# raphaelsty/mkb

Hardware: AMD Instinct MI355X
Metric: scored triples/sec (pos+K neg), FB15k-237 RotatE d=1000 (higher is better)
Workload: dtype f32

## Files before the change

### mkb_amd/csrc/score_pool_tile.h

```cpp
#pragma once
#include "score_pool_kernels.h"

namespace mkb {

#ifndef MKB_TILE_KC
#define MKB_TILE_KC 16
#endif
#ifndef MKB_TILE_CP_PIPE
#define MKB_TILE_CP_PIPE 1
#endif
constexpr int kTileKC = MKB_TILE_KC;
constexpr int kTileNQ = kTileKC / 16;
constexpr int kTileRows = 64, kTilePos = 64;
constexpr int kTilePitch = kTileRows * 4 + 4;

struct TileArgs {
    float *part;
    int Kd, ks;
    int fringe_tiles, fringe_slices;
    int row_tiles, pos_tiles;
};

constexpr int kTileL2 = 16;
template <> struct ModelTraits<kTileL2> { static constexpr bool cplx_query = false, cplx_pair = false, uses_gamma = false; };

template <int MODEL, bool HEAD>
__device__ __forceinline__ f2 tile_pair_term(float4 q, float4 x) {
    if constexpr (ModelTraits<MODEL>::cplx_pair) {
        return pair_term_cmod2(f2{q.x, q.y}, f2{q.z, q.w}, f2{x.x, x.y}, f2{x.z, x.w});
    } else {
        static_assert(MODEL == MKB_TRANSE, "real-valued tile: TransE's |q - x| only");
        const f2 a = HEAD ? f2{x.x, x.y} + f2{q.x, q.y} : f2{q.x, q.y} - f2{x.x, x.y};
        const f2 b = HEAD ? f2{x.z, x.w} + f2{q.z, q.w} : f2{q.z, q.w} - f2{x.z, x.w};
        f2 r;
        asm("v_add_f32 %0, |%1|, |%2|" : "=v"(r.x) : "v"(a.x), "v"(b.x));
        asm("v_add_f32 %0, |%1|, |%2|" : "=v"(r.y) : "v"(a.y), "v"(b.y));
        return r;
    }
}

template <int MODEL, bool HEAD>
__device__ __forceinline__ void tile_pair_acc(f2 &acc, float4 q, float4 x) {
    if constexpr (MODEL == kTileL2) {
        const f2 a = f2{q.x, q.y} - f2{x.x, x.y};
        const f2 b = f2{q.z, q.w} - f2{x.z, x.w};
        acc = __builtin_elementwise_fma(b, b, __builtin_elementwise_fma(a, a, acc));
    } else {
        acc += tile_pair_term<MODEL, HEAD>(q, x);
    }
}

template <int MODEL, bool HEAD, int KPT>
__global__ __launch_bounds__(256) void pool_fwd_tile_kernel(PoolArgs A, TileArgs T) {
    constexpr bool CP = ModelTraits<MODEL>::cplx_pair;
    extern __shared__ __attribute__((aligned(16))) int lds_tile_dyn[];
    const int b = (int)blockIdx.x;
    const int n_fringe = T.fringe_tiles * T.fringe_slices;
    if constexpr (MODEL != kTileL2) {
        if (b < n_fringe) {
            pool_fwd_body<MODEL, HEAD, KPT, 4>(A, b % T.fringe_tiles, T.fringe_tiles, b / T.fringe_tiles, T.fringe_slices, lds_tile_dyn);
            return;
        }
    }
    __shared__ __attribute__((aligned(16))) float sq[2][kTileKC / 2][kTilePitch];
    __shared__ __attribute__((aligned(16))) float sx[2][kTileKC / 2][kTilePitch];
    int t = b - n_fringe;
    const int z = t % T.ks; t /= T.ks;
    const int i0 = (t % T.row_tiles) * kTileRows, p0 = (t / T.row_tiles) * kTilePos;
    const int tid = threadIdx.x, lane = tid & 63, wave = tid >> 6;
    const int lr = lane & 7, lp = lane >> 3;
    const int wr = (wave >> 1) * 32, wp = (wave & 1) * 32;
    const int d = CP ? A.d : (int)(A.De / 2);
    const int kper = ((d + T.ks - 1) / T.ks + kTileKC - 1) / kTileKC * kTileKC;
    const int k_lo = z * kper, k_hi = min(d, k_lo + kper);

    const int srow = tid >> 2, skq = tid & 3;
    const float *qsrc = A.Q + (int64_t)min(i0 + srow, A.B - 1) * A.De;
    const float *xsrc = A.ent + A.pool[min(p0 + srow, T.Kd - 1)] * A.De;
    float4 rq_re[kTileNQ], rq_im[kTileNQ], rx_re[kTileNQ], rx_im[kTileNQ];
    auto gload = [&](int k0) {
#pragma unroll
        for (int j = 0; j < kTileNQ; ++j) {
            const int kq = k0 + 4 * (skq + 4 * j);
            if constexpr (CP) {
                const int k = min(kq, d - 4);
                rq_re[j] = *reinterpret_cast<const float4 *>(qsrc + k);
                rq_im[j] = *reinterpret_cast<const float4 *>(qsrc + d + k);
                rx_re[j] = *reinterpret_cast<const float4 *>(xsrc + k);
                rx_im[j] = *reinterpret_cast<const float4 *>(xsrc + d + k);
            } else {
                const int f0 = min(2 * kq, (int)A.De - 4), f1 = min(2 * kq + 4, (int)A.De - 4);
                rq_re[j] = *reinterpret_cast<const float4 *>(qsrc + f0);
                rq_im[j] = *reinterpret_cast<const float4 *>(qsrc + f1);
                rx_re[j] = *reinterpret_cast<const float4 *>(xsrc + f0);
                rx_im[j] = *reinterpret_cast<const float4 *>(xsrc + f1);
            }
        }
    };
    auto lstore = [&](int buf, int k0) {
        const float4 zz = make_float4(0.f, 0.f, 0.f, 0.f);
#pragma unroll
        for (int j = 0; j < kTileNQ; ++j) {
            const int kq = k0 + 4 * (skq + 4 * j), g0 = 2 * (skq + 4 * j);
            if constexpr (CP) {
                const bool ok = kq < k_hi;
                const float4 a = ok ? rq_re[j] : zz, bq = ok ? rq_im[j] : zz, c = ok ? rx_re[j] : zz, e = ok ? rx_im[j] : zz;
                *reinterpret_cast<float4 *>(&sq[buf][g0][srow * 4]) = make_float4(a.x, a.y, bq.x, bq.y);
                *reinterpret_cast<float4 *>(&sq[buf][g0 + 1][srow * 4]) = make_float4(a.z, a.w, bq.z, bq.w);
                *reinterpret_cast<float4 *>(&sx[buf][g0][srow * 4]) = make_float4(c.x, c.y, e.x, e.y);
                *reinterpret_cast<float4 *>(&sx[buf][g0 + 1][srow * 4]) = make_float4(c.z, c.w, e.z, e.w);
            } else {
                const bool ok0 = kq < k_hi, ok1 = kq + 2 < k_hi;
                *reinterpret_cast<float4 *>(&sq[buf][g0][srow * 4]) = ok0 ? rq_re[j] : zz;
                *reinterpret_cast<float4 *>(&sq[buf][g0 + 1][srow * 4]) = ok1 ? rq_im[j] : zz;
                *reinterpret_cast<float4 *>(&sx[buf][g0][srow * 4]) = ok0 ? rx_re[j] : zz;
                *reinterpret_cast<float4 *>(&sx[buf][g0 + 1][srow * 4]) = ok1 ? rx_im[j] : zz;
            }
        }
    };
    f2 acc[4][4];
#pragma unroll
    for (int a = 0; a < 4; ++a)
#pragma unroll
        for (int c = 0; c < 4; ++c) acc[a][c] = f2{0.f, 0.f};
    if (k_lo < k_hi) {
        gload(k_lo);
        lstore(0, k_lo);
    }
    __syncthreads();
    int buf = 0;
    for (int k0 = k_lo; k0 < k_hi; k0 += kTileKC) {
        const bool more = k0 + kTileKC < k_hi;
        if (more) gload(k0 + kTileKC);
        if constexpr (CP && MKB_TILE_CP_PIPE == 0) {
#pragma unroll 1
            for (int kp = 0; kp < kTileKC / 2; ++kp) {
                float4 q[4], x[4];
#pragma unroll
                for (int a = 0; a < 4; ++a) q[a] = *reinterpret_cast<const float4 *>(&sq[buf][kp][(wr + lr + 8 * a) * 4]);
#pragma unroll
                for (int c = 0; c < 4; ++c) x[c] = *reinterpret_cast<const float4 *>(&sx[buf][kp][(wp + lp + 8 * c) * 4]);
#pragma unroll
                for (int a = 0; a < 4; ++a)
#pragma unroll
                    for (int c = 0; c < 4; ++c)
                        tile_pair_acc<MODEL, HEAD>(acc[a][c], q[a], x[c]);
            }
        } else {
            float4 qa[4], xa[4], qb[4], xb[4];
            auto lds_group = [&](int kp, float4 (&q)[4], float4 (&x)[4]) {
#pragma unroll
                for (int a = 0; a < 4; ++a) q[a] = *reinterpret_cast<const float4 *>(&sq[buf][kp][(wr + lr + 8 * a) * 4]);
#pragma unroll
                for (int c = 0; c < 4; ++c) x[c] = *reinterpret_cast<const float4 *>(&sx[buf][kp][(wp + lp + 8 * c) * 4]);
            };
            auto terms = [&](const float4 (&q)[4], const float4 (&x)[4]) {
#pragma unroll
                for (int a = 0; a < 4; ++a)
#pragma unroll
                    for (int c = 0; c < 4; ++c) tile_pair_acc<MODEL, HEAD>(acc[a][c], q[a], x[c]);
            };
            lds_group(0, qa, xa);
#pragma unroll 1
            for (int kp = 0; kp < kTileKC / 2; kp += 2) {
                lds_group(kp + 1, qb, xb);
                terms(qa, xa);
                lds_group(min(kp + 2, kTileKC / 2 - 1), qa, xa);
                terms(qb, xb);
            }
        }
        if (more) lstore(buf ^ 1, k0 + kTileKC);
        __syncthreads();
        buf ^= 1;
    }
    float *out = T.part + (int64_t)z * A.B * T.Kd;
#pragma unroll
    for (int a = 0; a < 4; ++a) {
        const int i = i0 + wr + lr + 8 * a;
#pragma unroll
        for (int c = 0; c < 4; ++c) {
            const int p = p0 + wp + lp + 8 * c;
            if (i < A.B && p < T.Kd) out[(int64_t)i * T.Kd + p] = acc[a][c].x + acc[a][c].y;
        }
    }
}

template <int UNUSED = 0>
__global__ __launch_bounds__(256) void tile_scores_reduce_kernel(const float *__restrict__ part, const uint16_t *__restrict__ cnt,
                                                                 float *__restrict__ S, int B, int P, int Kd, int ks, float c0, float c1) {
    const int64_t n = (int64_t)B * Kd;
    for (int64_t e = (int64_t)blockIdx.x * 256 + threadIdx.x; e < n; e += (int64_t)gridDim.x * 256) {
        const int64_t i = e / Kd, p = e - i * Kd;
        float s = 0.f;
        for (int z0 = 0; z0 < ks; z0 += 8) {
            float v[8];
#pragma unroll
            for (int k = 0; k < 8; ++k) v[k] = part[(int64_t)min(z0 + k, ks - 1) * n + e];
#pragma unroll
            for (int k = 0; k < 8; ++k) s += z0 + k < ks ? v[k] : 0.f;
        }
        S[i * P + p] = cnt[i * P + p] ? c0 + c1 * s : 0.f;
    }
}

template <int MODEL, bool HEAD>
static int launch_fwd_tile(const PoolLaunch &L, const PoolArgs &A0, hipStream_t st, float *part, GemmTail *tail) {
    if constexpr (!ModelTraits<MODEL>::cplx_pair && MODEL != MKB_TRANSE) {
        return set_error(MKB_ERR_UNSUPPORTED, "pool_fwd_tile: complex-modulus pair function and TransE only");
    } else {
        PoolArgs A = A0;
        TileArgs T{};
        T.part = part; T.Kd = L.tile_kd; T.ks = L.tile_ks;
        T.row_tiles = (A.B + kTileRows - 1) / kTileRows; T.pos_tiles = T.Kd / kTilePos;
        A.p_lo = T.Kd;
        const bool fringe = A.P > T.Kd;
        T.fringe_tiles = fringe ? (A.B + TI - 1) / TI : 0;
        T.fringe_slices = fringe ? L.tile_fringe_slices : 0;
        const size_t lds = (T.fringe_tiles > 0) ? (size_t)3 * ((A.P - T.Kd + T.fringe_slices - 1) / T.fringe_slices) * 4 : 0;
        const unsigned blocks = (unsigned)(T.fringe_tiles * T.fringe_slices + T.row_tiles * T.pos_tiles * T.ks);
        if (L.fkpt == 4) hipLaunchKernelGGL((pool_fwd_tile_kernel<MODEL, HEAD, 4>), dim3(blocks), dim3(256), lds, st, A, T);
        else hipLaunchKernelGGL((pool_fwd_tile_kernel<MODEL, HEAD, 2>), dim3(blocks), dim3(256), lds, st, A, T);
        if (tail) {
            *tail = GemmTail{3, part, A.S, nullptr, A.B, T.Kd, T.ks, A.P, (int64_t)A.B * T.Kd, A.c0, A.c1, nullptr, 0};
        } else {
            hipLaunchKernelGGL(tile_scores_reduce_kernel<0>, dim3(512), dim3(256), 0, st, part, A.cnt, A.S, A.B, A.P, T.Kd, T.ks, A.c0, A.c1);
        }
        MKB_LAUNCH_CHECK();
        return MKB_OK;
    }
}

}
```

Baseline: 1.206 billion.

## Stage tile epilogue through LDS for float4 stores and reorder prologue loads

The tile scoring kernel now writes its 4x4 per-thread accumulators into a padded LDS image and then writes each row to global memory as coalesced float4s, replacing scattered scalar stores. The prologue issues the query loads before the entity row is resolved through the pool index, to hide the dependent index lookup. The main loop is split so the last chunk runs without the per-iteration 'more' branch. The epilogue reuses the staging buffers and adds one extra barrier, and a misaligned or non-multiple-of-four Kd falls back to scalar stores.

New measurement: 1.193 billion (median of 3 runs). No clear change (-1.1%).

```diff
diff --git a/mkb_amd/csrc/score_pool_tile.h b/mkb_amd/csrc/score_pool_tile.h
--- a/mkb_amd/csrc/score_pool_tile.h
+++ b/mkb_amd/csrc/score_pool_tile.h
@@ -8,11 +8,21 @@
 #endif
 #ifndef MKB_TILE_CP_PIPE
 #define MKB_TILE_CP_PIPE 1
+#endif
+#ifndef MKB_TILE_EPI_LDS
+#define MKB_TILE_EPI_LDS 1
+#endif
+#ifndef MKB_TILE_LOADS_AHEAD
+#define MKB_TILE_LOADS_AHEAD 1
+#endif
+#ifndef MKB_TILE_Q_FIRST
+#define MKB_TILE_Q_FIRST 1
 #endif
 constexpr int kTileKC = MKB_TILE_KC;
 constexpr int kTileNQ = kTileKC / 16;
 constexpr int kTileRows = 64, kTilePos = 64;
 constexpr int kTilePitch = kTileRows * 4 + 4;
+constexpr int kTileEpiPitch = 36;
 
 struct TileArgs {
     float *part;
@@ -76,9 +86,8 @@
 
     const int srow = tid >> 2, skq = tid & 3;
     const float *qsrc = A.Q + (int64_t)min(i0 + srow, A.B - 1) * A.De;
-    const float *xsrc = A.ent + A.pool[min(p0 + srow, T.Kd - 1)] * A.De;
     float4 rq_re[kTileNQ], rq_im[kTileNQ], rx_re[kTileNQ], rx_im[kTileNQ];
-    auto gload = [&](int k0) {
+    auto gload_q = [&](int k0) {
 #pragma unroll
         for (int j = 0; j < kTileNQ; ++j) {
             const int kq = k0 + 4 * (skq + 4 * j);
@@ -86,12 +95,23 @@
                 const int k = min(kq, d - 4);
                 rq_re[j] = *reinterpret_cast<const float4 *>(qsrc + k);
                 rq_im[j] = *reinterpret_cast<const float4 *>(qsrc + d + k);
+            } else {
+                const int f0 = min(2 * kq, (int)A.De - 4), f1 = min(2 * kq + 4, (int)A.De - 4);
+                rq_re[j] = *reinterpret_cast<const float4 *>(qsrc + f0);
+                rq_im[j] = *reinterpret_cast<const float4 *>(qsrc + f1);
+            }
+        }
+    };
+    auto gload_x = [&](const float *xsrc, int k0) {
+#pragma unroll
+        for (int j = 0; j < kTileNQ; ++j) {
+            const int kq = k0 + 4 * (skq + 4 * j);
+            if constexpr (CP) {
+                const int k = min(kq, d - 4);
                 rx_re[j] = *reinterpret_cast<const float4 *>(xsrc + k);
                 rx_im[j] = *reinterpret_cast<const float4 *>(xsrc + d + k);
             } else {
                 const int f0 = min(2 * kq, (int)A.De - 4), f1 = min(2 * kq + 4, (int)A.De - 4);
-                rq_re[j] = *reinterpret_cast<const float4 *>(qsrc + f0);
-                rq_im[j] = *reinterpret_cast<const float4 *>(qsrc + f1);
                 rx_re[j] = *reinterpret_cast<const float4 *>(xsrc + f0);
                 rx_im[j] = *reinterpret_cast<const float4 *>(xsrc + f1);
             }
@@ -123,15 +143,26 @@
     for (int a = 0; a < 4; ++a)
 #pragma unroll
         for (int c = 0; c < 4; ++c) acc[a][c] = f2{0.f, 0.f};
-    if (k_lo < k_hi) {
-        gload(k_lo);
+    const int64_t *pid = A.pool + min(p0 + srow, T.Kd - 1);
+    const float *xsrc;
+    if constexpr (MKB_TILE_Q_FIRST != 0) {
+        const int64_t e = *pid;
+        gload_q(k_lo);
+        asm volatile("" ::: "memory");
+        xsrc = A.ent + e * A.De;
+        gload_x(xsrc, k_lo);
         lstore(0, k_lo);
+    } else {
+        xsrc = A.ent + *pid * A.De;
+        if (k_lo < k_hi) {
+            gload_q(k_lo);
+            gload_x(xsrc, k_lo);
+            lstore(0, k_lo);
+        }
     }
     __syncthreads();
     int buf = 0;
-    for (int k0 = k_lo; k0 < k_hi; k0 += kTileKC) {
-        const bool more = k0 + kTileKC < k_hi;
-        if (more) gload(k0 + kTileKC);
+    auto chunk_math = [&](int buf) {
         if constexpr (CP && MKB_TILE_CP_PIPE == 0) {
 #pragma unroll 1
             for (int kp = 0; kp < kTileKC / 2; ++kp) {
@@ -169,18 +200,68 @@
                 terms(qb, xb);
             }
         }
-        if (more) lstore(buf ^ 1, k0 + kTileKC);
+    };
+    if constexpr (MKB_TILE_LOADS_AHEAD != 0) {
+        for (int k0 = k_lo; k0 + kTileKC < k_hi; k0 += kTileKC) {
+            gload_q(k0 + kTileKC);
+            gload_x(xsrc, k0 + kTileKC);
+            chunk_math(buf);
+            lstore(buf ^ 1, k0 + kTileKC);
+            __syncthreads();
+            buf ^= 1;
+        }
+        if (k_lo < k_hi) chunk_math(buf);
         __syncthreads();
-        buf ^= 1;
+    } else {
+        for (int k0 = k_lo; k0 < k_hi; k0 += kTileKC) {
+            const bool more = k0 + kTileKC < k_hi;
+            if (more) {
+                gload_q(k0 + kTileKC);
+                gload_x(xsrc, k0 + kTileKC);
+            }
+            chunk_math(buf);
+            if (more) lstore(buf ^ 1, k0 + kTileKC);
+            __syncthreads();
+            buf ^= 1;
+        }
     }
     float *out = T.part + (int64_t)z * A.B * T.Kd;
-#pragma unroll
-    for (int a = 0; a < 4; ++a) {
-        const int i = i0 + wr + lr + 8 * a;
-#pragma unroll
-        for (int c = 0; c < 4; ++c) {
-            const int p = p0 + wp + lp + 8 * c;
-            if (i < A.B && p < T.Kd) out[(int64_t)i * T.Kd + p] = acc[a][c].x + acc[a][c].y;
+    if constexpr (MKB_TILE_EPI_LDS != 0) {
+        static_assert(2 * 32 * kTileEpiPitch <= 2 * (kTileKC / 2) * kTilePitch, "two waves' epilogue images fit one staging array");
+        float *ep = (wave < 2 ? &sq[0][0][0] : &sx[0][0][0]) + (wave & 1) * 32 * kTileEpiPitch;
+#pragma unroll
+        for (int a = 0; a < 4; ++a)
+#pragma unroll
+            for (int c = 0; c < 4; ++c) ep[(lr + 8 * a) * kTileEpiPitch + lp + 8 * c] = acc[a][c].x + acc[a][c].y;
+        __syncthreads();
+        const int er = lane >> 3, p = p0 + wp + (lane & 7) * 4;
+        float4 v[4];
+#pragma unroll
+        for (int j = 0; j < 4; ++j) v[j] = *reinterpret_cast<const float4 *>(&ep[(er + 8 * j) * kTileEpiPitch + (lane & 7) * 4]);
+        const bool quads = (T.Kd & 3) == 0 && ((uintptr_t)out & 15) == 0;
+        float *o = out + (int64_t)(i0 + wr + er) * T.Kd + p;
+        if (quads) {
+#pragma unroll
+            for (int j = 0; j < 4; ++j)
+                if (i0 + wr + er + 8 * j < A.B && p < T.Kd) *reinterpret_cast<float4 *>(o + (int64_t)8 * j * T.Kd) = v[j];
+        } else {
+#pragma unroll
+            for (int j = 0; j < 4; ++j) {
+                const float e[4] = {v[j].x, v[j].y, v[j].z, v[j].w};
+#pragma unroll
+                for (int c = 0; c < 4; ++c)
+                    if (i0 + wr + er + 8 * j < A.B && p + c < T.Kd) o[(int64_t)8 * j * T.Kd + c] = e[c];
+            }
+        }
+    } else {
+#pragma unroll
+        for (int a = 0; a < 4; ++a) {
+            const int i = i0 + wr + lr + 8 * a;
+#pragma unroll
+            for (int c = 0; c < 4; ++c) {
+                const int p = p0 + wp + lp + 8 * c;
+                if (i < A.B && p < T.Kd) out[(int64_t)i * T.Kd + p] = acc[a][c].x + acc[a][c].y;
+            }
         }
     }
 }
```
